# jynik/OOKiedokie

Hardware: NVIDIA B200
Metric: IQ Msamples/s decoded (SC16Q11->OOK msgs) (higher is better)
Workload: dtype f32

## Files before the change

### include/ookd_gpu.h

```cpp
#ifndef OOKD_GPU_H
#define OOKD_GPU_H

#include <stddef.h>
#include <stdint.h>

#ifdef __cplusplus
extern "C" {
#endif

#define OOKD_MAX_STAGES   8
#define OOKD_MAX_TAPS     1024
#define OOKD_MSG_BYTES    32

#define OOKD_OK             0
#define OOKD_ERR_ARG       (-1)
#define OOKD_ERR_CUDA      (-2)
#define OOKD_ERR_NOMEM     (-3)
#define OOKD_ERR_STATE     (-4)
#define OOKD_ERR_OVERFLOW  (-5)

struct ookd_filter_desc {
    uint32_t num_stages;
    uint32_t decimation[OOKD_MAX_STAGES];
    uint32_t num_taps[OOKD_MAX_STAGES];
// ... 38 lines not shown
};

struct ookd_sm_state_k {
    uint32_t first_trigger, num_triggers;
    uint32_t dmin, dmax;
    uint32_t ktimeout;
    uint32_t ksat;
};

struct ookd_sm_compiled {
    uint32_t num_states, num_triggers;
    struct ookd_sm_state_k   *states;
    struct ookd_sm_trigger_k *triggers;
    uint32_t max_bits;
    uint32_t k_sat;
};

int  ookd_sm_compile(const struct ookd_sm_desc *desc, struct ookd_sm_compiled *out);
void ookd_sm_compiled_free(struct ookd_sm_compiled *c);

float ookd_power_threshold(float thr);

extern const int16_t ookd_tune_quarter[257];
int ookd_tune_step(double offset_hz, uint32_t samplerate, uint32_t *step);
int ookd_tune_sc16q11(const int16_t *in, int16_t *out, uint64_t first_sample, uint64_t n_samples, uint32_t step);

struct ookd_msg {
    uint64_t out_sample;
    uint64_t buffer_idx;
    uint32_t num_bits;
    uint32_t reserved;
    uint8_t  data[OOKD_MSG_BYTES];
};

struct ookd_sm_carry {
    uint32_t state;
    uint32_t k;
    uint32_t num_bits;
    uint32_t prev_bit;
    uint8_t  data[OOKD_MSG_BYTES];
};

void ookd_sm_idle_carry(const struct ookd_sm_compiled *c, struct ookd_sm_carry *out);

struct ookd_gpu_config {
    const struct ookd_filter_desc *filter;
    const struct ookd_sm_desc *sm;
    float    threshold;
    uint32_t samples_per_buffer;
    int32_t  device_id;
    uint32_t flags;
    uint32_t sm_chunk_buffers;
    uint32_t sm_warmup;
    uint32_t sm_burst_rounds;
    uint32_t sub_windows;
    uint32_t tune_step;
};

// ... 131 lines not shown
```

### ookiedokie_b200/binding.py

```python
import ctypes as C
import os
import subprocess

import numpy as np

_HERE = os.path.dirname(os.path.abspath(__file__))
LIB_PATH = os.environ.get("OOKD_GPU_LIB") or os.path.join(_HERE, "lib", "libookd_gpu.so")

MAX_STAGES = 8
MSG_BYTES = 32
K_INF = 0xFFFFFFFF

FLAG_FORCE_GENERIC = 1
FLAG_NO_SCREEN = 2
FLAG_NO_TMA = 8
FLAG_SYNC_TAIL = 16
FLAG_SHARE_SMS = 32
FLAG_NO_GRAPH = 64
FLAG_FUSED_SM = 128
FLAG_FMA_SCREEN = 256
FLAG_NO_ADAPTIVE = 512
FLAG_INPUT_CS8 = 1024
FLAG_INPUT_CU8 = 2048

INPUT_FORMATS = {"sc16q11": (0, np.int16), "cs8": (FLAG_INPUT_CS8, np.int8), "cu8": (FLAG_INPUT_CU8, np.uint8)}

EXPORTS = [
    "ookd_sm_compile", "ookd_sm_compiled_free", "ookd_sm_idle_carry", "ookd_power_threshold",
    "ookd_tune_step", "ookd_tune_sc16q11",
    "ookd_gpu_device_count", "ookd_gpu_strerror", "ookd_gpu_last_error",
    "ookd_gpu_create", "ookd_gpu_destroy", "ookd_gpu_decode", "ookd_gpu_decode_shard",
    "ookd_gpu_decode_begin", "ookd_gpu_decode_end", "ookd_gpu_batch_decode",
    "ookd_gpu_resolve", "ookd_gpu_halo", "ookd_gpu_input_bytes", "ookd_gpu_total_decimation", "ookd_gpu_initial_carry",
    "ookd_gpu_edges", "ookd_gpu_bits", "ookd_gpu_filtered", "ookd_gpu_filter_cf", "ookd_gpu_synth", "ookd_gpu_synth_ex",
    "ookd_gpu_host_alloc", "ookd_gpu_host_free", "ookd_gpu_dev_alloc", "ookd_gpu_dev_free",
    "ookd_gpu_memcpy_h2d", "ookd_gpu_memcpy_d2h", "ookd_gpu_filtered_sc16q11",
    "ookd_gpu_multi_create", "ookd_gpu_multi_destroy", "ookd_gpu_multi_halo", "ookd_gpu_multi_n_gpus",
    "ookd_gpu_multi_handle", "ookd_gpu_multi_shards_used", "ookd_gpu_multi_last_error", "ookd_gpu_multi_shard_range",
    "ookd_gpu_multi_decode", "ookd_gpu_multi_edges",
    "ookd_gpu_multi_decode_begin", "ookd_gpu_multi_decode_end", "ookd_gpu_multi_resolve",
]


# ... 25 lines not shown


class SmTriggerK(C.Structure):
    _fields_ = [("cond", C.c_int32), ("action", C.c_int32), ("next_state", C.c_uint32),
                ("kmin", C.c_uint32), ("kmax", C.c_uint32)]


class SmStateK(C.Structure):
    _fields_ = [("first_trigger", C.c_uint32), ("num_triggers", C.c_uint32),
                ("dmin", C.c_uint32), ("dmax", C.c_uint32), ("ktimeout", C.c_uint32), ("ksat", C.c_uint32)]


class SmCompiled(C.Structure):
    _fields_ = [("num_states", C.c_uint32), ("num_triggers", C.c_uint32),
                ("states", C.POINTER(SmStateK)), ("triggers", C.POINTER(SmTriggerK)),
                ("max_bits", C.c_uint32), ("k_sat", C.c_uint32)]


class Msg(C.Structure):
    _fields_ = [("out_sample", C.c_uint64), ("buffer_idx", C.c_uint64), ("num_bits", C.c_uint32),
                ("reserved", C.c_uint32), ("data", C.c_uint8 * MSG_BYTES)]


MSG_DTYPE = np.dtype([("out_sample", "<u8"), ("buffer_idx", "<u8"), ("num_bits", "<u4"), ("reserved", "<u4"),
                      ("data", "u1", (MSG_BYTES,))])
assert MSG_DTYPE.itemsize == C.sizeof(Msg)


def msgs_to_tuples(rec, nbytes):
    return list(zip(rec["out_sample"].tolist(), rec["buffer_idx"].tolist(), rec["num_bits"].tolist(),
                    [bytes(d[:nbytes]) for d in rec["data"]]))
# ... 39 lines not shown


_lib = None


def lib():
    global _lib
    if _lib is None:
        if not os.path.exists(LIB_PATH):
            build_library()
        L = C.CDLL(LIB_PATH)
        L.ookd_sm_compile.restype = C.c_int
        L.ookd_sm_compile.argtypes = [C.POINTER(SmDesc), C.POINTER(SmCompiled)]
        L.ookd_sm_compiled_free.argtypes = [C.POINTER(SmCompiled)]
        L.ookd_sm_idle_carry.argtypes = [C.POINTER(SmCompiled), C.POINTER(SmCarry)]
        L.ookd_power_threshold.restype = C.c_float
        L.ookd_power_threshold.argtypes = [C.c_float]
        L.ookd_tune_step.restype = C.c_int
        L.ookd_tune_step.argtypes = [C.c_double, C.c_uint32, C.POINTER(C.c_uint32)]
        L.ookd_tune_sc16q11.restype = C.c_int
        L.ookd_tune_sc16q11.argtypes = [C.c_void_p, C.c_void_p, C.c_uint64, C.c_uint64, C.c_uint32]
        L.ookd_gpu_device_count.restype = C.c_int
        L.ookd_gpu_strerror.restype = C.c_char_p
        L.ookd_gpu_strerror.argtypes = [C.c_int]
        L.ookd_gpu_last_error.restype = C.c_char_p
        L.ookd_gpu_last_error.argtypes = [C.c_void_p]
        L.ookd_gpu_create.restype = C.c_int
        L.ookd_gpu_create.argtypes = [C.POINTER(C.c_void_p), C.POINTER(GpuConfig)]
        L.ookd_gpu_destroy.argtypes = [C.c_void_p]
        L.ookd_gpu_decode.restype = C.c_int
# ... 130 lines not shown
    return res


def sm_idle_carry(states, num_bits, sample_rate):
    d, keep = make_sm_desc(states, num_bits, sample_rate)
    out = SmCompiled()
    rc = lib().ookd_sm_compile(C.byref(d), C.byref(out))
    if rc != 0:
        raise OokdError(f"ookd_sm_compile: {lib().ookd_gpu_strerror(rc).decode()}")
    c = SmCarry()
    lib().ookd_sm_idle_carry(C.byref(out), C.byref(c))
    lib().ookd_sm_compiled_free(C.byref(out))
    return c.astuple()


def power_threshold(thr):
    return float(lib().ookd_power_threshold(C.c_float(thr)))


def tune_step(offset_hz, samplerate):
    if not 0 <= int(samplerate) < 2**32:
        raise ValueError(f"samplerate {samplerate} is not a uint32")
    step = C.c_uint32()
    if lib().ookd_tune_step(C.c_double(float(offset_hz)), C.c_uint32(int(samplerate)), C.byref(step)) != 0:
        raise ValueError(f"no tune step for an offset of {offset_hz} Hz at {samplerate} samples/s: the offset must be "
                         f"finite and below half the sample rate in magnitude")
    return int(step.value)


def tune_sc16q11(iq, first_sample, step):
# ... 334 lines not shown
```

### ookiedokie_b200/csrc/ookd_gpu.cu

```cuda
#include <cstdarg>
#include <cstdio>
#include <cstdlib>
#include <cmath>
#include <algorithm>
#include <cstring>
#include <mutex>
#include <thread>
#include <type_traits>
#include <vector>

#include "ookd_common.cuh"
#include "fir_kernels.cuh"
#include "screen_tma.cuh"
#include "edge_kernels.cuh"
#include "sm_kernels.cuh"
#include "synth_kernel.cuh"

using namespace ookd;

namespace {

struct DevBuf {
    void  *p = nullptr;
    size_t cap = 0;
// ... 51 lines not shown
    uint32_t tune_step = 0;
    bool screen = false;
    bool screen2 = false;
    bool fma = false;
    bool fma_ok = false;
    bool adaptive = false;
    bool adaptive_ok = false;
    bool fused_sm = true;
    unsigned fused_grid_max = 0;
    unsigned n_sm = 148;

    bool have_sm = false;
    ookd_sm_compiled smc{};
    SmCarry canon{};
    SmTable *d_tab = nullptr;

    DevBuf in, bits, inter[2], block_counts, edges, scalars, chunk_exit[2], chunk_ran, slots, slot_count,
           sm_dbg, slot_off, msgs_dev, dense_list, chunk_e, bound_pos, seed_pos, seed_e, seed_kind, edge_tmp, final_entry, tab_entry, tab_exit, tab_nmsg, tab_cnt[2], tab_link, tab_chosen;
    uint32_t slot_cap = 8;
    bool tables_valid = false;
    int tab_cur = 0;
    bool warmup = false;
    u64 warm_in = 0;
    bool warm = false;
    i64 report_lo = 0;
    SmCarry entry_used{};
    uint32_t first_chunk = 0;
    bool entry_explicit = false;
    void *h_scalars = nullptr;
    SmMsg *h_msgs_pin = nullptr;
// ... 534 lines not shown
        o.buffer_idx = ((m.out_sample + 1) * (u64) h->total_dec - 1) / h->spb;
        o.num_bits = m.num_bits;
        memcpy(o.data, m.data, nbytes);
    }
    if (exit_) carry_from_dev(last, *exit_);
    if (res) {
        res->n_msgs = h->h_msgs.size();
        res->msgs = h->h_msgs.empty() ? nullptr : h->h_msgs.data();
        res->sm_rounds = rounds;
        carry_from_dev(h->entry_used, res->entry_used);
        res->entry_is_provisional = (h->warm && !h->entry_explicit) ? 1u : 0u;
    }
    return OOKD_OK;
}

SmArgs base_sm_args(ookd_gpu *h, const SmCarry &entry0)
{
    SmArgs a{};
    a.tab = h->d_tab;
    a.edges = (const u64 *) h->edges.p;
    a.n_edges = h->n_edges;
    a.base_bit = h->base_bit;
    a.out_lo = h->out_lo; a.out_hi = h->out_hi;
    a.spb = h->spb; a.dec = h->total_dec;
    a.opb = (h->spb % h->total_dec == 0) ? h->spb / h->total_dec : 0;
    a.first_buffer = h->first_buffer;
    a.chunk_buffers = h->chunk_buffers;
    a.n_chunks = h->n_chunks;
    a.entry0 = entry0;
    a.slots = (SmMsg *) h->slots.p;
    a.slot_cap = h->slot_cap;
    a.n_ran = (uint32_t *) ((char *) h->scalars.p + 64);
    a.overflow = (uint32_t *) ((char *) h->scalars.p + 32);
    a.warm = h->warm ? 1u : 0u;
// ... 208 lines not shown
            for (uint32_t r = 0; r < burst; r++) {
                a.round = rounds;
                a.counter_idx = rounds & 31;
                if (rounds == 0) {
                    a.cnt_in = (const uint32_t *) h->tab_cnt[0].p;
                    a.cnt_out = (uint32_t *) h->tab_cnt[0].p;
                } else {
                    CU(h, cudaMemcpyAsync(h->tab_cnt[cur ^ 1].p, h->tab_cnt[cur].p, sizeof(uint32_t) * nc,
                                          cudaMemcpyDeviceToDevice, h->s_compute));
                    a.cnt_in = (const uint32_t *) h->tab_cnt[cur].p;
                    a.cnt_out = (uint32_t *) h->tab_cnt[cur ^ 1].p;
                    cur ^= 1;
                }
                {
                    const u64 warps = (u64) nc * (rounds == 0 ? 1 : TAB_K);
                    sm_table_round_kernel<<<(unsigned) ((warps + SM_ROUND_WARPS - 1) / SM_ROUND_WARPS), 32 * SM_ROUND_WARPS, 0, h->s_compute>>>(a);
                }
                h->launches++;
                CU(h, cudaGetLastError());
                rounds++;
                if (burst == 3 && r <= 1) {
                    a.cnt_in = (const uint32_t *) h->tab_cnt[cur].p;
                    sm_link_kernel<<<(unsigned) (((u64) nc * TAB_K + 127) / 128), 128, 0, h->s_compute>>>(a);
                    sm_walk_kernel<<<1, SM_WALK_NT, 0, h->s_compute>>>(a, nullptr, nullptr, 0, nullptr);
                    h->launches += 2;
                }
            }
            a.cnt_in = (const uint32_t *) h->tab_cnt[cur].p;
            sm_link_kernel<<<(unsigned) (((u64) nc * TAB_K + 127) / 128), 128, 0, h->s_compute>>>(a);
            sm_walk_kernel<<<1, SM_WALK_NT, 0, h->s_compute>>>(a, nullptr, nullptr, 0, nullptr);
            h->launches += 2;
// ... 204 lines not shown
    h->launches++;
    for (uint32_t r = 0; r < h->burst_rounds; r++) {
        a.round = rounds;
        a.counter_idx = rounds & 31;
        if (rounds == 0) {
            a.cnt_in = (const uint32_t *) h->tab_cnt[0].p;
            a.cnt_out = (uint32_t *) h->tab_cnt[0].p;
        } else {
            CU(h, cudaMemcpyAsync(h->tab_cnt[cur ^ 1].p, h->tab_cnt[cur].p, sizeof(uint32_t) * nc, cudaMemcpyDeviceToDevice,
                                  h->s_compute));
            a.cnt_in = (const uint32_t *) h->tab_cnt[cur].p;
            a.cnt_out = (uint32_t *) h->tab_cnt[cur ^ 1].p;
            cur ^= 1;
        }
        const u64 warps = (u64) nc * (rounds == 0 ? 1 : TAB_K);
        sm_table_round_kernel<<<(unsigned) ((warps + SM_ROUND_WARPS - 1) / SM_ROUND_WARPS), 32 * SM_ROUND_WARPS, 0, h->s_compute>>>(a);
        h->launches++;
        CU(h, cudaGetLastError());
        rounds++;
        {
            a.cnt_in = (const uint32_t *) h->tab_cnt[cur].p;
            sm_link_kernel<<<(unsigned) (((u64) nc * TAB_K + 127) / 128), 128, 0, h->s_compute>>>(a);
            sm_walk_kernel<<<1, SM_WALK_NT, 0, h->s_compute>>>(a, (uint32_t *) h->slot_off.p, (SmMsg *) h->msgs_dev.p, msg_cap,
                                                               (u64 *) h->scalars.p + 1);
            h->launches += 2;
        }
    }
    }
    CU(h, cudaGetLastError());
    CU(h, cudaMemcpyAsync(h->h_scalars, h->scalars.p, 352, cudaMemcpyDeviceToHost, h->s_compute));
    if (getenv("OOKD_DEBUG")) {
// ... 136 lines not shown
                us(0), us(1), us(2), us(8), us(9), us(3), us(4), us(5), us(7), rounds, nc);
    }
    if (!h->fused_sm && !h->burst_fixed && overflow == 0 && walk_complete != 1 && h->burst_rounds < 2) {
        h->burst_rounds = 2;
    }
    while (!h->fused_sm && overflow == 0 && walk_complete != 1 && rounds < 16) {
        SmArgs a = fast_sm_args(h, h->pend.e0);
        a.round = rounds;
        a.counter_idx = rounds & 15;
        CU(h, cudaMemcpyAsync(h->tab_cnt[cur ^ 1].p, h->tab_cnt[cur].p, sizeof(uint32_t) * nc, cudaMemcpyDeviceToDevice,
                              h->s_compute));
        a.cnt_in = (const uint32_t *) h->tab_cnt[cur].p;
        a.cnt_out = (uint32_t *) h->tab_cnt[cur ^ 1].p;
        cur ^= 1;
        const u64 warps = (u64) nc * TAB_K;
        sm_table_round_kernel<<<(unsigned) ((warps + SM_ROUND_WARPS - 1) / SM_ROUND_WARPS), 32 * SM_ROUND_WARPS, 0, h->s_compute>>>(a);
        rounds++;
        a.cnt_in = (const uint32_t *) h->tab_cnt[cur].p;
        sm_link_kernel<<<(unsigned) (((u64) nc * TAB_K + 127) / 128), 128, 0, h->s_compute>>>(a);
        sm_walk_kernel<<<1, SM_WALK_NT, 0, h->s_compute>>>(a, nullptr, nullptr, 0, nullptr);
        CU(h, cudaMemcpyAsync(h->slot_off.p, h->slot_count.p, sizeof(uint32_t) * nc, cudaMemcpyDeviceToDevice, h->s_compute));
        scan_u32_kernel<<<1, SCAN_NT, 0, h->s_compute>>>((uint32_t *) h->slot_off.p, nc, (u64 *) h->scalars.p + 1);
        sm_gather_table_kernel<<<(nc + 127) / 128, 128, 0, h->s_compute>>>(a, (const uint32_t *) h->slot_off.p,
                                                                           (SmMsg *) h->msgs_dev.p, msg_cap);
        h->launches += 5;
        CU(h, cudaGetLastError());
        CU(h, cudaMemcpyAsync(h->h_scalars, h->scalars.p, 352, cudaMemcpyDeviceToHost, h->s_compute));
        if (n_copy) {
            CU(h, cudaMemcpyAsync(h->h_msgs_pin, h->msgs_dev.p, sizeof(SmMsg) * n_copy, cudaMemcpyDeviceToHost, h->s_compute));
        }
        if (h->warm) {
// ... 68 lines not shown
    return h ? h->err : "null handle";
}

void ookd_gpu_destroy(ookd_gpu *h)
{
    if (!h) return;
    if (h->sub) ookd_gpu_multi_destroy(h->sub);
    h->sub = nullptr;
    cudaSetDevice(h->device);
    if (h->s_compute) cudaStreamSynchronize(h->s_compute);
    if (h->s_copy) cudaStreamSynchronize(h->s_copy);
    if (h->tail_graph) cudaGraphExecDestroy(h->tail_graph);
    h->tail_graph = nullptr;
    for (auto &st : h->stages) if (st.d_taps) cudaFree(st.d_taps);
    if (h->d_tab) cudaFree(h->d_tab);
    DevBuf *all[] = {&h->in, &h->bits, &h->inter[0], &h->inter[1], &h->block_counts, &h->edges, &h->scalars,
                     &h->chunk_exit[0], &h->chunk_exit[1], &h->chunk_ran, &h->slots, &h->slot_count,
                     &h->sm_dbg, &h->slot_off, &h->msgs_dev, &h->dense_list, &h->chunk_e, &h->bound_pos, &h->seed_pos, &h->seed_e, &h->seed_kind, &h->edge_tmp,
                     &h->final_entry, &h->tab_entry, &h->tab_exit, &h->tab_nmsg, &h->tab_cnt[0],
                     &h->tab_cnt[1], &h->tab_link, &h->tab_chosen};
    for (DevBuf *b : all) release(*b);
    if (h->h_scalars) cudaFreeHost(h->h_scalars);
    if (h->h_msgs_pin) cudaFreeHost(h->h_msgs_pin);
    for (auto e : h->ev_piece) cudaEventDestroy(e);
    if (h->ev_t0) cudaEventDestroy(h->ev_t0);
    if (h->ev_t1) cudaEventDestroy(h->ev_t1);
    if (h->ev_f0) cudaEventDestroy(h->ev_f0);
    if (h->ev_f1) cudaEventDestroy(h->ev_f1);
    if (h->ev_s1) cudaEventDestroy(h->ev_s1);
    if (h->s_compute) cudaStreamDestroy(h->s_compute);
// ... 145 lines not shown
        }
        const int rc = ookd_sm_compile(cfg->sm, &h->smc);
        if (rc != OOKD_OK) CREATE_FAIL(rc);
        SmTable *tab = new SmTable();
        memset(tab, 0, sizeof(*tab));
        tab->num_states = h->smc.num_states;
        tab->num_triggers = h->smc.num_triggers;
        tab->max_bits = h->smc.max_bits;
        tab->k_sat = h->smc.k_sat;
        memcpy(tab->states, h->smc.states, sizeof(ookd_sm_state_k) * h->smc.num_states);
        memcpy(tab->triggers, h->smc.triggers, sizeof(ookd_sm_trigger_k) * h->smc.num_triggers);
        cudaError_t e = cudaMalloc(&h->d_tab, sizeof(SmTable));
        if (e == cudaSuccess) e = cudaMemcpy(h->d_tab, tab, sizeof(SmTable), cudaMemcpyHostToDevice);
        delete tab;
        if (e != cudaSuccess) CREATE_FAIL(OOKD_ERR_CUDA);
        ookd_sm_carry idle;
        ookd_sm_idle_carry(&h->smc, &idle);
        carry_to_dev(idle, h->canon);
        h->have_sm = true;
    }
    if (cfg->sub_windows > 1 && cfg->sm) {
        const uint32_t K = cfg->sub_windows < 16 ? cfg->sub_windows : 16;
        ookd_gpu_config c = *cfg;
        c.sub_windows = 0;
        c.device_id = dev;
        int32_t ids[16];
        for (uint32_t k = 0; k < K; k++) ids[k] = dev;
        const int rc = ookd_gpu_multi_create(&h->sub, &c, ids, K);
        if (rc != OOKD_OK) CREATE_FAIL(rc);
        if (ookd_gpu_multi_halo(h->sub) != h->halo) CREATE_FAIL(OOKD_ERR_STATE);
// ... 606 lines not shown
```

### ookiedokie_b200/csrc/sm_compile.c

```c
#include "ookd_gpu.h"

#include <math.h>
#include <stdlib.h>
#include <string.h>

#define SM_TOLERANCE 0.15
#define K_LIMIT 0x7FFFFFF0u

struct bound {
    double   value;
    int      is_lower;
    uint32_t k;
    int      done;
};

static double win_lo(uint64_t d_us)
{
    const float lo = (float) ((double) d_us - (SM_TOLERANCE * (double) d_us));
    return (double) lo;
}

static double win_hi(uint64_t d_us)
{
    const float hi = (float) ((double) d_us + (SM_TOLERANCE * (double) d_us));
// ... 32 lines not shown
                    b[i].k = k;
                } else {
                    b[i].done = 1;
                    open--;
                }
            }
        }
        if (k >= K_LIMIT) {
            return OOKD_ERR_ARG;
        }
        elapsed += dt;
        k++;
    }
    return OOKD_OK;
}

int ookd_sm_compile(const struct ookd_sm_desc *d, struct ookd_sm_compiled *out)
{
    if (!d || !out || d->num_states == 0 || !d->states || d->max_bits == 0 ||
        d->max_bits > 8 * OOKD_MSG_BYTES || d->sample_rate == 0 ||
        (d->num_triggers != 0 && !d->triggers)) {
        return OOKD_ERR_ARG;
    }
    memset(out, 0, sizeof(*out));

    for (uint32_t s = 0; s < d->num_states; s++) {
        const struct ookd_sm_state_us *st = &d->states[s];
        if ((uint64_t) st->first_trigger + st->num_triggers > d->num_triggers) {
            return OOKD_ERR_ARG;
        }
// ... 86 lines not shown
        struct ookd_sm_state_k *o = &out->states[s];
        for (uint32_t t = 0; t < o->num_triggers; t++) {
            const struct ookd_sm_trigger_k *tk = &out->triggers[o->first_trigger + t];
            if (tk->kmax != OOKD_K_INF) {
                if (tk->kmin + 1 > o->ksat) o->ksat = tk->kmin + 1;
                if (tk->kmax + 1 > o->ksat) o->ksat = tk->kmax + 1;
            }
        }
    }
    free(b);

    out->num_states = d->num_states;
    out->num_triggers = d->num_triggers;
    out->max_bits = d->max_bits;
    out->k_sat = k_max + 1;
    return OOKD_OK;
}

void ookd_sm_compiled_free(struct ookd_sm_compiled *c)
{
    if (c) {
        free(c->states);
        free(c->triggers);
        memset(c, 0, sizeof(*c));
    }
}

float ookd_power_threshold(float thr)
{
    if (isnan(thr)) {
        return thr;
    }
    if (thr <= 0.0f) {
        return 0.0f;
    }
    if (isinf(thr)) {
        return INFINITY;
    }
    float p = thr * thr;
    if (isinf(p)) {
// ... 145 lines not shown
```

### ookiedokie_b200/csrc/sm_kernels.cuh

```cuda
#pragma once

#include "ookd_common.cuh"

namespace ookd {

struct SmDevHdr {
    u64 n_edges;
    uint32_t base_bit, pad;
};

struct SmArgs {
    const SmDevHdr *hdr;
    const SmTable *tab;
    const u64 *edges;
    u64  n_edges;
    uint32_t base_bit;
    i64  out_lo, out_hi;
    u64  spb;
    u64  dec;
    uint32_t opb;
    u64  first_buffer;
    uint32_t chunk_buffers;
    uint32_t n_chunks;
    uint32_t round;
// ... 21 lines not shown
    SmCarry  *final_exit;
    uint32_t *start_slot;
    uint32_t first_chunk;
    uint32_t warm;
    SmCarry  *final_entry;
    i64 report_lo;
    SmCarry  *mid_carry;
    unsigned long long *dbg;
    uint32_t entry_at_report;
    u64 *chunk_e;
    i64 *bound_pos;
    i64 *seed_pos;
    u64 *seed_e;
    uint8_t *seed_kind;
    SmCarry canon;
};

#define OOKD_SEED_TRUE      0
#define OOKD_SEED_CANON     1
#define OOKD_SEED_IDLE      2
#define OOKD_SEED_RESET     3
#define OOKD_SEED_NONE      4

__device__ __forceinline__ i64 first_output_of_buffer(const SmArgs &a, u64 b)
{
    if (a.opb) return (i64) (b * a.opb);
    return (i64) ((b * a.spb) / a.dec);
}

__device__ __forceinline__ u64 buffer_of_output(const SmArgs &a, i64 m)
// ... 300 lines not shown
    if (lane < tab->num_triggers) {
        const ookd_sm_trigger_k t = tab->triggers[lane];
        W.t_cond = (uint32_t) t.cond;
        W.t_pack = (uint32_t) t.action | (t.next_state << 8);
        W.t_kmin = t.kmin; W.t_kmax = t.kmax;
        for (uint32_t st = 0; st < tab->num_states; st++) {
            const ookd_sm_state_k x = tab->states[st];
            if (lane >= x.first_trigger && lane < x.first_trigger + x.num_triggers) {
                W.t_state = st;
                W.s_dmin = x.dmin; W.s_dmax = x.dmax; W.s_ktimeout = x.ktimeout; W.s_ksat = x.ksat;
            }
        }
    }
}

__device__ __forceinline__ int warp_sm_apply(const WarpSm &W, SmCarry &s, uint32_t pack)
{
    const uint32_t action = pack & 0xFFu;
    int result = 0;
    if (action == OOKD_ACT_APPEND_0 || action == OOKD_ACT_APPEND_1) {
        if (s.num_bits <= W.max_bits && s.num_bits < 256) {
            const u64 m = 1ull << (s.num_bits & 63);
            const u64 set = (action == OOKD_ACT_APPEND_1) ? m : 0ull;
            if (s.num_bits < 64) {
                s.data[0] = (s.data[0] & ~m) | set;
            } else {
                const uint32_t w = s.num_bits >> 6;
#pragma unroll
                for (uint32_t i = 1; i < 4; i++) {
                    if (i == w) s.data[i] = (s.data[i] & ~m) | set;
                }
            }
        }
        s.num_bits++;
    } else if (action == OOKD_ACT_OUTPUT_DATA) {
        result = 1;
    }
    s.state = pack >> 8;
    return result;
}

__device__ __forceinline__ int warp_sm_eval(const WarpSm &W, SmCarry &s, uint32_t b)
{
    const uint32_t k = s.k;
    const bool rise = !s.prev && b, fall = s.prev && !b;
    const bool cond_ok = (W.t_cond == OOKD_COND_ALWAYS) || (W.t_cond == OOKD_COND_PULSE_START && rise) ||
                         (W.t_cond == OOKD_COND_PULSE_END && fall) ||
                         (W.t_cond == OOKD_COND_TIMEOUT && W.s_ktimeout != OOKD_K_INF && k >= W.s_ktimeout) ||
                         (W.t_cond == OOKD_COND_MSG_COMPLETE && s.num_bits >= W.max_bits);
    const bool elig = (W.t_state == s.state) && k >= W.t_kmin && k <= W.t_kmax && cond_ok;
    const uint32_t mask = __ballot_sync(0xFFFFFFFFu, elig);
    if (mask == 0) {
        const uint32_t ksat = __shfl_sync(0xFFFFFFFFu, W.ksat_by_state, (int) s.state);
        s.k = (k + 1 < ksat) ? k + 1 : ksat;
// ... 550 lines not shown
    bool live = c < a.n_chunks;
    if (live && a.round != 0) live = (c != 0) && j < a.cnt_in[c - 1];
    if (threadIdx.x == 0) s_any = 0;
    __syncthreads();
    if (live && lane == 0) s_any = 1;
    __syncthreads();
    if (!s_any) return;
    load_table(T, a.tab);
    if (!live) return;
    const bool capable = warp_sm_supported(a.tab);
    WarpSm W;
    if (capable) warp_sm_load(W, &T, lane);
    sm_round_pair(a, T, W, capable, c, j, lane, n_edges, base_bit);
}

__global__ void __launch_bounds__(32) sm_table_add_entry_kernel(const SmArgs a)
{
    __shared__ SmTable T;
    load_table(T, a.tab);
    const uint32_t lane = threadIdx.x & 31;
    const uint32_t K = a.tab_k;
    const uint32_t c = a.first_chunk;
    const uint32_t n_here = a.cnt_out[c];
    SmCarry s = a.entry0;
    if (!a.entry_at_report) {
        for (uint32_t i = 0; i < n_here; i++) {
            if (carry_equal(s, a.tab_entry[(u64) c * K + i])) { if (lane == 0) *a.start_slot = i; return; }
        }
    } else {
        for (uint32_t i = 0; i < n_here; i++) {
// ... 417 lines not shown
```

Baseline: 1.001 million.

## Add precompiled breakpoint table and per-thread state machine evaluation

Compiles the OOK state machine into a per-state breakpoint table that gives, for each k interval, the quiet-fire time and the rising/falling edge outcomes. A new kernel runs one chunk/entry pair per thread, with the table copied into shared memory, instead of one warp per pair using ballot-based trigger evaluation. Long runs with no edge are skipped in a single step by jumping straight to the next fire time. This cuts per-sample and per-warp cost in the sequential state-machine rounds. In exchange, only one pair is packed per thread, which can cause divergence, and lookups add shared-memory traffic; machines with too many states or breakpoints fall back to the old warp path.

```diff
diff --git a/include/ookd_gpu.h b/include/ookd_gpu.h
--- a/include/ookd_gpu.h
+++ b/include/ookd_gpu.h
@@ -76,7 +76,15 @@
     struct ookd_sm_trigger_k *triggers;
     uint32_t max_bits;
     uint32_t k_sat;
-};
+    uint32_t *table;
+    uint32_t table_words;
+};
+
+#define OOKD_SMT_MAX_STATES 32
+#define OOKD_SMT_BP         16
+#define OOKD_SMT_ROW        (OOKD_SMT_BP * 9)
+#define OOKD_SMT_ERROR      0xFFFFFFFFu
+#define OOKD_SMT_MAX_WORDS  (OOKD_SMT_MAX_STATES * OOKD_SMT_ROW)
 
 int  ookd_sm_compile(const struct ookd_sm_desc *desc, struct ookd_sm_compiled *out);
 void ookd_sm_compiled_free(struct ookd_sm_compiled *c);
@@ -104,6 +112,9 @@
 };
 
 void ookd_sm_idle_carry(const struct ookd_sm_compiled *c, struct ookd_sm_carry *out);
+
+int ookd_sm_table_step(const struct ookd_sm_compiled *c, struct ookd_sm_carry *s, uint32_t b);
+uint32_t ookd_sm_table_quiet(const struct ookd_sm_compiled *c, const struct ookd_sm_carry *s, uint32_t *k_fire);
 
 struct ookd_gpu_config {
     const struct ookd_filter_desc *filter;
diff --git a/ookiedokie_b200/binding.py b/ookiedokie_b200/binding.py
--- a/ookiedokie_b200/binding.py
+++ b/ookiedokie_b200/binding.py
@@ -8,6 +8,9 @@
 LIB_PATH = os.environ.get("OOKD_GPU_LIB") or os.path.join(_HERE, "lib", "libookd_gpu.so")
 
 MAX_STAGES = 8
+SMT_BP = 16
+SMT_ROW = SMT_BP * 9
+SMT_ERROR = 0xFFFFFFFF
 MSG_BYTES = 32
 K_INF = 0xFFFFFFFF
 
@@ -26,7 +29,8 @@
 INPUT_FORMATS = {"sc16q11": (0, np.int16), "cs8": (FLAG_INPUT_CS8, np.int8), "cu8": (FLAG_INPUT_CU8, np.uint8)}
 
 EXPORTS = [
-    "ookd_sm_compile", "ookd_sm_compiled_free", "ookd_sm_idle_carry", "ookd_power_threshold",
+    "ookd_sm_compile", "ookd_sm_compiled_free", "ookd_sm_idle_carry", "ookd_sm_table_step", "ookd_sm_table_quiet",
+    "ookd_power_threshold",
     "ookd_tune_step", "ookd_tune_sc16q11",
     "ookd_gpu_device_count", "ookd_gpu_strerror", "ookd_gpu_last_error",
     "ookd_gpu_create", "ookd_gpu_destroy", "ookd_gpu_decode", "ookd_gpu_decode_shard",
@@ -82,7 +86,8 @@
 class SmCompiled(C.Structure):
     _fields_ = [("num_states", C.c_uint32), ("num_triggers", C.c_uint32),
                 ("states", C.POINTER(SmStateK)), ("triggers", C.POINTER(SmTriggerK)),
-                ("max_bits", C.c_uint32), ("k_sat", C.c_uint32)]
+                ("max_bits", C.c_uint32), ("k_sat", C.c_uint32),
+                ("table", C.POINTER(C.c_uint32)), ("table_words", C.c_uint32)]
 
 
 class Msg(C.Structure):
@@ -152,6 +157,10 @@
         L.ookd_sm_compile.argtypes = [C.POINTER(SmDesc), C.POINTER(SmCompiled)]
         L.ookd_sm_compiled_free.argtypes = [C.POINTER(SmCompiled)]
         L.ookd_sm_idle_carry.argtypes = [C.POINTER(SmCompiled), C.POINTER(SmCarry)]
+        L.ookd_sm_table_step.restype = C.c_int
+        L.ookd_sm_table_step.argtypes = [C.POINTER(SmCompiled), C.POINTER(SmCarry), C.c_uint32]
+        L.ookd_sm_table_quiet.restype = C.c_uint32
+        L.ookd_sm_table_quiet.argtypes = [C.POINTER(SmCompiled), C.POINTER(SmCarry), C.POINTER(C.c_uint32)]
         L.ookd_power_threshold.restype = C.c_float
         L.ookd_power_threshold.argtypes = [C.c_float]
         L.ookd_tune_step.restype = C.c_int
@@ -312,6 +321,41 @@
     return c.astuple()
 
 
+class CompiledSm:
+
+    def __init__(self, states, num_bits, sample_rate):
+        d, keep = make_sm_desc(states, num_bits, sample_rate)
+        self.c = SmCompiled()
+        rc = lib().ookd_sm_compile(C.byref(d), C.byref(self.c))
+        if rc != 0:
+            self.c = None
+            raise OokdError(f"ookd_sm_compile: {lib().ookd_gpu_strerror(rc).decode()}")
+
+    def table(self):
+        if not self.c.table:
+            return None
+        return np.ctypeslib.as_array(self.c.table, shape=(self.c.table_words,)).copy().reshape(self.c.num_states, -1)
+
+    def ksat(self, s):
+        return self.c.states[s].ksat
+
+    def step(self, carry, b):
+        x = SmCarry.fromtuple(carry)
+        r = lib().ookd_sm_table_step(C.byref(self.c), C.byref(x), int(b))
+        return r, x.astuple()
+
+    def quiet(self, carry):
+        x = SmCarry.fromtuple(carry)
+        k = C.c_uint32(0)
+        pack = lib().ookd_sm_table_quiet(C.byref(self.c), C.byref(x), C.byref(k))
+        return pack, k.value
+
+    def __del__(self):
+        if getattr(self, "c", None) is not None and lib is not None:
+            lib().ookd_sm_compiled_free(C.byref(self.c))
+            self.c = None
+
+
 def power_threshold(thr):
     return float(lib().ookd_power_threshold(C.c_float(thr)))
 
diff --git a/ookiedokie_b200/csrc/ookd_gpu.cu b/ookiedokie_b200/csrc/ookd_gpu.cu
--- a/ookiedokie_b200/csrc/ookd_gpu.cu
+++ b/ookiedokie_b200/csrc/ookd_gpu.cu
@@ -89,6 +89,9 @@
     ookd_sm_compiled smc{};
     SmCarry canon{};
     SmTable *d_tab = nullptr;
+    uint32_t *d_smt = nullptr;
+    uint32_t smt_words = 0;
+    uint32_t smt_ppw = 32;
 
     DevBuf in, bits, inter[2], block_counts, edges, scalars, chunk_exit[2], chunk_ran, slots, slot_count,
            sm_dbg, slot_off, msgs_dev, dense_list, chunk_e, bound_pos, seed_pos, seed_e, seed_kind, edge_tmp, final_entry, tab_entry, tab_exit, tab_nmsg, tab_cnt[2], tab_link, tab_chosen;
@@ -653,10 +656,23 @@
     return OOKD_OK;
 }
 
+void launch_round(ookd_gpu *h, const SmArgs &a, u64 pairs)
+{
+    if (h->d_smt) {
+        sm_thread_round_kernel<<<(unsigned) ((pairs + a.smt_ppw - 1) / a.smt_ppw), SM_THREAD_NT,
+                                 sizeof(uint32_t) * h->smt_words, h->s_compute>>>(a);
+    } else {
+        sm_table_round_kernel<<<(unsigned) ((pairs + SM_ROUND_WARPS - 1) / SM_ROUND_WARPS), 32 * SM_ROUND_WARPS, 0, h->s_compute>>>(a);
+    }
+}
+
 SmArgs base_sm_args(ookd_gpu *h, const SmCarry &entry0)
 {
     SmArgs a{};
     a.tab = h->d_tab;
+    a.smt = h->d_smt;
+    a.smt_words = h->smt_words;
+    a.smt_ppw = h->smt_ppw;
     a.edges = (const u64 *) h->edges.p;
     a.n_edges = h->n_edges;
     a.base_bit = h->base_bit;
@@ -895,7 +911,7 @@
                 }
                 {
                     const u64 warps = (u64) nc * (rounds == 0 ? 1 : TAB_K);
-                    sm_table_round_kernel<<<(unsigned) ((warps + SM_ROUND_WARPS - 1) / SM_ROUND_WARPS), 32 * SM_ROUND_WARPS, 0, h->s_compute>>>(a);
+                    launch_round(h, a, warps);
                 }
                 h->launches++;
                 CU(h, cudaGetLastError());
@@ -1130,7 +1146,7 @@
             cur ^= 1;
         }
         const u64 warps = (u64) nc * (rounds == 0 ? 1 : TAB_K);
-        sm_table_round_kernel<<<(unsigned) ((warps + SM_ROUND_WARPS - 1) / SM_ROUND_WARPS), 32 * SM_ROUND_WARPS, 0, h->s_compute>>>(a);
+        launch_round(h, a, warps);
         h->launches++;
         CU(h, cudaGetLastError());
         rounds++;
@@ -1297,7 +1313,7 @@
         a.cnt_out = (uint32_t *) h->tab_cnt[cur ^ 1].p;
         cur ^= 1;
         const u64 warps = (u64) nc * TAB_K;
-        sm_table_round_kernel<<<(unsigned) ((warps + SM_ROUND_WARPS - 1) / SM_ROUND_WARPS), 32 * SM_ROUND_WARPS, 0, h->s_compute>>>(a);
+        launch_round(h, a, warps);
         rounds++;
         a.cnt_in = (const uint32_t *) h->tab_cnt[cur].p;
         sm_link_kernel<<<(unsigned) (((u64) nc * TAB_K + 127) / 128), 128, 0, h->s_compute>>>(a);
@@ -1396,6 +1412,7 @@
     h->tail_graph = nullptr;
     for (auto &st : h->stages) if (st.d_taps) cudaFree(st.d_taps);
     if (h->d_tab) cudaFree(h->d_tab);
+    if (h->d_smt) cudaFree(h->d_smt);
     DevBuf *all[] = {&h->in, &h->bits, &h->inter[0], &h->inter[1], &h->block_counts, &h->edges, &h->scalars,
                      &h->chunk_exit[0], &h->chunk_exit[1], &h->chunk_ran, &h->slots, &h->slot_count,
                      &h->sm_dbg, &h->slot_off, &h->msgs_dev, &h->dense_list, &h->chunk_e, &h->bound_pos, &h->seed_pos, &h->seed_e, &h->seed_kind, &h->edge_tmp,
@@ -1571,6 +1588,17 @@
         if (e == cudaSuccess) e = cudaMemcpy(h->d_tab, tab, sizeof(SmTable), cudaMemcpyHostToDevice);
         delete tab;
         if (e != cudaSuccess) CREATE_FAIL(OOKD_ERR_CUDA);
+        const char *ev = getenv("OOKD_SM_EVAL");
+        if (h->smc.table && !(ev && strcmp(ev, "warp") == 0)) {
+            e = cudaMalloc(&h->d_smt, sizeof(uint32_t) * h->smc.table_words);
+            if (e == cudaSuccess) {
+                e = cudaMemcpy(h->d_smt, h->smc.table, sizeof(uint32_t) * h->smc.table_words, cudaMemcpyHostToDevice);
+            }
+            if (e != cudaSuccess) CREATE_FAIL(OOKD_ERR_CUDA);
+            h->smt_words = h->smc.table_words;
+            const char *ppw = getenv("OOKD_SM_PPW");
+            if (ppw && atoi(ppw) >= 1 && atoi(ppw) <= 32) h->smt_ppw = (uint32_t) atoi(ppw);
+        }
         ookd_sm_carry idle;
         ookd_sm_idle_carry(&h->smc, &idle);
         carry_to_dev(idle, h->canon);
diff --git a/ookiedokie_b200/csrc/sm_compile.c b/ookiedokie_b200/csrc/sm_compile.c
--- a/ookiedokie_b200/csrc/sm_compile.c
+++ b/ookiedokie_b200/csrc/sm_compile.c
@@ -70,6 +70,8 @@
     }
     return OOKD_OK;
 }
+
+static int build_table(struct ookd_sm_compiled *c);
 
 int ookd_sm_compile(const struct ookd_sm_desc *d, struct ookd_sm_compiled *out)
 {
@@ -186,6 +188,10 @@
     out->num_triggers = d->num_triggers;
     out->max_bits = d->max_bits;
     out->k_sat = k_max + 1;
+    if (build_table(out) != OOKD_OK) {
+        ookd_sm_compiled_free(out);
+        return OOKD_ERR_NOMEM;
+    }
     return OOKD_OK;
 }
 
@@ -194,8 +200,209 @@
     if (c) {
         free(c->states);
         free(c->triggers);
+        free(c->table);
         memset(c, 0, sizeof(*c));
     }
+}
+
+
+static uint32_t tab_outcome(const struct ookd_sm_compiled *c, uint32_t s, uint32_t k, uint32_t prev, uint32_t b, int mc)
+{
+    const struct ookd_sm_state_k *st = &c->states[s];
+    for (uint32_t i = 0; i < st->num_triggers; i++) {
+        const struct ookd_sm_trigger_k *t = &c->triggers[st->first_trigger + i];
+        if (k < t->kmin || k > t->kmax) {
+            continue;
+        }
+        int fire = 0, check = 0;
+        switch (t->cond) {
+            case OOKD_COND_ALWAYS:       fire = 1; break;
+            case OOKD_COND_PULSE_START:  fire = check = (!prev && b); break;
+            case OOKD_COND_PULSE_END:    fire = check = (prev && !b); break;
+            case OOKD_COND_TIMEOUT:      fire = (st->ktimeout != OOKD_K_INF && k >= st->ktimeout); break;
+            case OOKD_COND_MSG_COMPLETE: fire = mc; break;
+            default: break;
+        }
+        if (fire) {
+            if (check && !(k >= st->dmin && k <= st->dmax)) {
+                return OOKD_SMT_ERROR;
+            }
+            return (uint32_t) t->action | (t->next_state << 8);
+        }
+    }
+    return 0;
+}
+
+static uint32_t tab_quiet(const struct ookd_sm_compiled *c, uint32_t s, uint32_t k, int mc, uint32_t *L)
+{
+    const struct ookd_sm_state_k *st = &c->states[s];
+    uint32_t best_k = OOKD_K_INF, pack = 0;
+    for (uint32_t i = 0; i < st->num_triggers; i++) {
+        const struct ookd_sm_trigger_k *t = &c->triggers[st->first_trigger + i];
+        uint32_t lo = t->kmin;
+        if (t->cond == OOKD_COND_TIMEOUT) {
+            if (st->ktimeout == OOKD_K_INF) continue;
+            if (st->ktimeout > lo) lo = st->ktimeout;
+        } else if (t->cond == OOKD_COND_MSG_COMPLETE) {
+            if (!mc) continue;
+        } else if (t->cond != OOKD_COND_ALWAYS) {
+            continue;
+        }
+        const uint32_t kk = lo > k ? lo : k;
+        if (kk > t->kmax) continue;
+        if (kk < best_k) {
+            best_k = kk;
+            pack = (uint32_t) t->action | (t->next_state << 8);
+        }
+    }
+    *L = best_k;
+    return pack;
+}
+
+static void bp_add(uint32_t *bp, uint32_t *n, uint32_t v, uint32_t ksat)
+{
+    if (v == 0 || v > ksat || v == OOKD_K_INF) {
+        return;
+    }
+    for (uint32_t i = 0; i < *n; i++) {
+        if (bp[i] == v) return;
+    }
+    if (*n < 2 * 32 + 4) {
+        bp[(*n)++] = v;
+    }
+}
+
+static int cmp_u32(const void *x, const void *y)
+{
+    const uint32_t a = *(const uint32_t *) x, b = *(const uint32_t *) y;
+    return (a > b) - (a < b);
+}
+
+static int build_table(struct ookd_sm_compiled *c)
+{
+    c->table = NULL;
+    c->table_words = 0;
+    if (c->num_states > OOKD_SMT_MAX_STATES || c->num_triggers > 32) {
+        return OOKD_OK;
+    }
+    uint32_t *tab = malloc(sizeof(uint32_t) * OOKD_SMT_ROW * c->num_states);
+    if (!tab) {
+        return OOKD_ERR_NOMEM;
+    }
+    for (uint32_t s = 0; s < c->num_states; s++) {
+        const struct ookd_sm_state_k *st = &c->states[s];
+        uint32_t bp[2 * 32 + 4], n = 0;
+        const uint32_t ksat = st->ksat;
+        bp_add(bp, &n, st->ktimeout, ksat);
+        bp_add(bp, &n, st->dmin, ksat);
+        if (st->dmax != OOKD_K_INF) bp_add(bp, &n, st->dmax + 1, ksat);
+        for (uint32_t i = 0; i < st->num_triggers; i++) {
+            const struct ookd_sm_trigger_k *t = &c->triggers[st->first_trigger + i];
+            bp_add(bp, &n, t->kmin, ksat);
+            if (t->kmax != OOKD_K_INF) bp_add(bp, &n, t->kmax + 1, ksat);
+        }
+        if (n > OOKD_SMT_BP - 1) {
+            free(tab);
+            return OOKD_OK;
+        }
+        qsort(bp, n, sizeof(bp[0]), cmp_u32);
+        uint32_t *row = tab + (size_t) s * OOKD_SMT_ROW;
+        row[0] = ksat;
+        for (uint32_t j = 1; j < OOKD_SMT_BP; j++) {
+            row[j] = (j - 1 < n) ? bp[j - 1] : OOKD_K_INF;
+        }
+        for (uint32_t i = 0; i < OOKD_SMT_BP; i++) {
+            uint32_t *o = row + OOKD_SMT_BP + 8 * i;
+            if (i > n) {
+                memset(o, 0, 8 * sizeof(uint32_t));
+                continue;
+            }
+            const uint32_t k = (i == 0) ? 0 : bp[i - 1];
+            for (int mc = 0; mc < 2; mc++) {
+                uint32_t L;
+                const uint32_t pack = tab_quiet(c, s, k, mc, &L);
+                o[2 * mc] = pack ? L : OOKD_K_INF;
+                o[2 * mc + 1] = pack;
+                o[4 + mc] = tab_outcome(c, s, k, 0, 1, mc);
+                o[6 + mc] = tab_outcome(c, s, k, 1, 0, mc);
+            }
+        }
+    }
+    c->table = tab;
+    c->table_words = OOKD_SMT_ROW * c->num_states;
+    return OOKD_OK;
+}
+
+static const uint32_t *tab_interval(const struct ookd_sm_compiled *c, uint32_t s, uint32_t k)
+{
+    const uint32_t *row = c->table + (size_t) s * OOKD_SMT_ROW;
+    uint32_t i = 0;
+    for (uint32_t j = 1; j < OOKD_SMT_BP; j++) {
+        i += (row[j] <= k);
+    }
+    return row + OOKD_SMT_BP + 8 * i;
+}
+
+static int tab_eval(const struct ookd_sm_compiled *c, struct ookd_sm_carry *s, uint32_t b)
+{
+    const uint32_t *o = tab_interval(c, s->state, s->k);
+    const int mc = s->num_bits >= c->max_bits;
+    uint32_t pack;
+    if ((s->prev_bit & 1u) == b) {
+        pack = (o[2 * mc] <= s->k) ? o[2 * mc + 1] : 0;
+    } else {
+        pack = o[(b ? 4 : 6) + mc];
+    }
+    if (pack == 0) {
+        const uint32_t ksat = c->table[(size_t) s->state * OOKD_SMT_ROW];
+        s->k = (s->k + 1 < ksat) ? s->k + 1 : ksat;
+        return 0;
+    }
+    s->k = 0;
+    if (pack == OOKD_SMT_ERROR) {
+        s->state = 0;
+        return -1;
+    }
+    const uint32_t action = pack & 0xFFu;
+    int result = 0;
+    if (action == OOKD_ACT_APPEND_0 || action == OOKD_ACT_APPEND_1) {
+        if (s->num_bits <= c->max_bits && s->num_bits < 8 * OOKD_MSG_BYTES) {
+            const uint32_t byte = s->num_bits >> 3, bit = s->num_bits & 7;
+            if (action == OOKD_ACT_APPEND_1) s->data[byte] |= (uint8_t) (1u << bit);
+            else s->data[byte] &= (uint8_t) ~(1u << bit);
+        }
+        s->num_bits++;
+    } else if (action == OOKD_ACT_OUTPUT_DATA) {
+        result = 1;
+    }
+    s->state = pack >> 8;
+    return result;
+}
+
+int ookd_sm_table_step(const struct ookd_sm_compiled *c, struct ookd_sm_carry *s, uint32_t b)
+{
+    int r = 0;
+    b &= 1u;
+    if (s->state == 0) {
+        const uint32_t nbytes = (c->max_bits + 7) / 8;
+        s->num_bits = 0;
+        memset(s->data, 0, nbytes < OOKD_MSG_BYTES ? nbytes : OOKD_MSG_BYTES);
+        r = tab_eval(c, s, b);
+    }
+    if (r == 0) {
+        r = tab_eval(c, s, b);
+    }
+    s->prev_bit = b;
+    return r;
+}
+
+uint32_t ookd_sm_table_quiet(const struct ookd_sm_compiled *c, const struct ookd_sm_carry *s, uint32_t *k_fire)
+{
+    const uint32_t *o = tab_interval(c, s->state, s->k);
+    const int mc = s->num_bits >= c->max_bits;
+    const uint32_t L = o[2 * mc], pack = o[2 * mc + 1];
+    *k_fire = pack ? (L > s->k ? L : s->k) : OOKD_K_INF;
+    return pack;
 }
 
 float ookd_power_threshold(float thr)
diff --git a/ookiedokie_b200/csrc/sm_kernels.cuh b/ookiedokie_b200/csrc/sm_kernels.cuh
--- a/ookiedokie_b200/csrc/sm_kernels.cuh
+++ b/ookiedokie_b200/csrc/sm_kernels.cuh
@@ -59,6 +59,9 @@
     u64 *seed_e;
     uint8_t *seed_kind;
     SmCarry canon;
+    const uint32_t *smt;
+    uint32_t smt_words;
+    uint32_t smt_ppw;
 };
 
 #define OOKD_SEED_TRUE      0
@@ -389,12 +392,12 @@
     }
 }
 
-__device__ __forceinline__ int warp_sm_apply(const WarpSm &W, SmCarry &s, uint32_t pack)
+__device__ __forceinline__ int sm_apply_pack(const uint32_t max_bits, SmCarry &s, uint32_t pack)
 {
     const uint32_t action = pack & 0xFFu;
     int result = 0;
     if (action == OOKD_ACT_APPEND_0 || action == OOKD_ACT_APPEND_1) {
-        if (s.num_bits <= W.max_bits && s.num_bits < 256) {
+        if (s.num_bits <= max_bits && s.num_bits < 256) {
             const u64 m = 1ull << (s.num_bits & 63);
             const u64 set = (action == OOKD_ACT_APPEND_1) ? m : 0ull;
             if (s.num_bits < 64) {
@@ -413,6 +416,11 @@
     }
     s.state = pack >> 8;
     return result;
+}
+
+__device__ __forceinline__ int warp_sm_apply(const WarpSm &W, SmCarry &s, uint32_t pack)
+{
+    return sm_apply_pack(W.max_bits, s, pack);
 }
 
 __device__ __forceinline__ int warp_sm_eval(const WarpSm &W, SmCarry &s, uint32_t b)
@@ -993,6 +1001,402 @@
     sm_round_pair(a, T, W, capable, c, j, lane, n_edges, base_bit);
 }
 
+struct SmtRow {
+    uint32_t w[OOKD_SMT_BP];
+};
+
+__device__ __forceinline__ void smt_row(const uint32_t *smt, uint32_t state, SmtRow &r)
+{
+    const uint4 *p = (const uint4 *) (smt + state * OOKD_SMT_ROW);
+#pragma unroll
+    for (int i = 0; i < OOKD_SMT_BP / 4; i++) {
+        const uint4 v = p[i];
+        r.w[4 * i] = v.x; r.w[4 * i + 1] = v.y; r.w[4 * i + 2] = v.z; r.w[4 * i + 3] = v.w;
+    }
+}
+
+__device__ __forceinline__ uint32_t smt_interval(const SmtRow &r, uint32_t k)
+{
+    uint32_t i = 0;
+#pragma unroll
+    for (int j = 1; j < OOKD_SMT_BP; j++) i += (r.w[j] <= k) ? 1u : 0u;
+    return i;
+}
+
+__device__ __forceinline__ int thr_sm_eval(const uint32_t *smt, uint32_t max_bits, SmCarry &s, uint32_t b)
+{
+    SmtRow r;
+    smt_row(smt, s.state, r);
+    const uint32_t k = s.k;
+    const uint32_t mc = (s.num_bits >= max_bits) ? 1u : 0u;
+    const uint32_t *o = smt + s.state * OOKD_SMT_ROW + OOKD_SMT_BP + 8 * smt_interval(r, k);
+    uint32_t pack;
+    if (s.prev == b) {
+        const uint2 q = *(const uint2 *) (o + 2 * mc);
+        pack = (q.x <= k) ? q.y : 0u;
+    } else {
+        pack = o[(b ? 4 : 6) + mc];
+    }
+    if (pack == 0) {
+        s.k = (k + 1 < r.w[0]) ? k + 1 : r.w[0];
+        return 0;
+    }
+    s.k = 0;
+    if (pack == OOKD_SMT_ERROR) {
+        s.state = 0;
+        return -1;
+    }
+    return sm_apply_pack(max_bits, s, pack);
+}
+
+__device__ __forceinline__ int thr_sm_step(const uint32_t *smt, uint32_t max_bits, SmCarry &s, uint32_t b)
+{
+    int r = 0;
+    if (s.state == 0) {
+        s.num_bits = 0;
+        const uint32_t nbytes = (max_bits + 7) >> 3;
+#pragma unroll
+        for (int w = 0; w < 4; w++) {
+            const uint32_t lo = 8u * w;
+            if (nbytes >= lo + 8) {
+                s.data[w] = 0;
+            } else if (nbytes > lo) {
+                s.data[w] &= ~((1ull << (8 * (nbytes - lo))) - 1);
+            }
+        }
+        r = thr_sm_eval(smt, max_bits, s, b);
+    }
+    if (r == 0) {
+        r = thr_sm_eval(smt, max_bits, s, b);
+    }
+    s.prev = b;
+    return r;
+}
+
+struct ThrEdges {
+    const u64 *edges;
+    u64 n_edges, ebase, org;
+    uint32_t A[8];
+    u64 R[8];
+
+    __device__ __forceinline__ uint32_t off(u64 v) const
+    {
+        const u64 d = v - org;
+        return d < 0xFFFFFFFFull ? (uint32_t) d : 0xFFFFFFFFu;
+    }
+    __device__ __forceinline__ void fetch8(u64 idx, u64 (&r)[8]) const
+    {
+        if (idx + 8 <= n_edges) {
+            const ulonglong2 *p = (const ulonglong2 *) (edges + idx);
+#pragma unroll
+            for (int i = 0; i < 4; i++) {
+                const ulonglong2 v = p[i];
+                r[2 * i] = v.x;
+                r[2 * i + 1] = v.y;
+            }
+        } else {
+#pragma unroll
+            for (int i = 0; i < 8; i++) r[i] = (idx + i < n_edges) ? edges[idx + i] : org + 0xFFFFFFFFull;
+        }
+    }
+    __device__ __forceinline__ void reset(u64 e)
+    {
+        ebase = e & ~1ull;
+        fetch8(ebase, R);
+#pragma unroll
+        for (int i = 0; i < 8; i++) A[i] = off(R[i]);
+        fetch8(ebase + 8, R);
+    }
+    __device__ __forceinline__ uint32_t at(u64 e)
+    {
+        if (e - ebase >= 8) {
+            if (e - ebase >= 16) {
+                reset(e);
+            } else {
+#pragma unroll
+                for (int i = 0; i < 8; i++) A[i] = off(R[i]);
+                ebase += 8;
+                fetch8(ebase + 8, R);
+            }
+        }
+        const uint32_t d = (uint32_t) (e - ebase);
+        uint32_t v = A[0];
+#pragma unroll
+        for (int i = 1; i < 8; i++) v = (d == (uint32_t) i) ? A[i] : v;
+        return v;
+    }
+    __device__ __forceinline__ u64 first_at_or_after(u64 e, uint32_t nb, u64 nb64)
+    {
+        if (e - ebase < 16) {
+            const uint32_t d = (uint32_t) (e - ebase);
+            uint32_t n = 0;
+#pragma unroll
+            for (int i = 0; i < 8; i++) {
+                n += ((uint32_t) i >= d && A[i] < nb ? 1u : 0u) + ((uint32_t) i + 8 >= d && off(R[i]) < nb ? 1u : 0u);
+            }
+            if (off(R[7]) >= nb) return e + n;
+            const u64 from = ebase + 16;
+            return from + edge_lower_bound_near(edges + from, n_edges - from, nb64);
+        }
+        return e + edge_lower_bound_near(edges + e, n_edges - e, nb64);
+    }
+};
+
+__device__ __forceinline__ void thr_sm_run_span(const SmArgs &a, const u64 n_edges, const uint32_t *smt, const uint32_t max_bits,
+                                                SmCarry &s, i64 pos64, i64 end64, u64 e, uint32_t tb, SpanOut &o, i64 chunk_lo)
+{
+    uint32_t pos = (uint32_t) (pos64 - chunk_lo);
+    const uint32_t end = (uint32_t) (end64 - chunk_lo);
+    ThrEdges E;
+    E.edges = a.edges; E.n_edges = n_edges; E.org = (u64) chunk_lo;
+    E.reset(e);
+    uint32_t next_edge = E.at(e);
+
+    if (s.prev & OOKD_CARRY_DROPPING) {
+        s.prev &= 1u;
+        i64 nb64 = next_buffer_start(a, pos64, chunk_lo);
+        const bool more = nb64 > end64;
+        if (more) nb64 = end64;
+        const uint32_t nb = (uint32_t) (nb64 - chunk_lo);
+        if (next_edge < nb) {
+            const u64 e2 = E.first_at_or_after(e, nb, (u64) nb64);
+            tb ^= (uint32_t) ((e2 - e) & 1);
+            e = e2;
+            next_edge = E.at(e);
+        }
+        pos = nb;
+        if (more) s.prev |= OOKD_CARRY_DROPPING;
+    }
+
+    while (pos < end) {
+        o.steps++;
+        int r;
+        if (s.state == 0 || s.prev != tb) {
+            const bool at_edge = (next_edge == pos);
+            const uint32_t b = at_edge ? (tb ^ 1u) : tb;
+            o.singles++;
+            r = thr_sm_step(smt, max_bits, s, b);
+            if (at_edge) {
+                tb ^= 1u;
+                e++;
+                next_edge = E.at(e);
+            }
+            pos++;
+        } else {
+            const bool have_edge = next_edge < end;
+            const uint32_t limit = have_edge ? next_edge : end;
+            const uint32_t g = limit - pos;
+            const uint32_t k = s.k;
+            const uint32_t b = tb ^ 1u;
+            SmtRow row;
+            smt_row(smt, s.state, row);
+            const uint32_t ksat = row.w[0];
+            const uint32_t k_e = min(k + g, ksat);
+            const uint32_t mc = (s.num_bits >= max_bits) ? 1u : 0u;
+            const uint32_t *o8 = smt + s.state * OOKD_SMT_ROW + OOKD_SMT_BP;
+            const uint2 q = *(const uint2 *) (o8 + 8 * smt_interval(row, k) + 2 * mc);
+            const uint32_t ew = o8[8 * smt_interval(row, k_e) + (b ? 4 : 6) + mc];
+            const uint32_t tau = max(q.x, k) - k;
+            if (q.y != 0 && tau < g) {
+                pos += tau + 1;
+                s.k = 0;
+                r = sm_apply_pack(max_bits, s, q.y);
+            } else if (!have_edge || ew == 0) {
+                const u64 kn = (u64) k + g + (have_edge ? 1u : 0u);
+                s.k = (kn < (u64) ksat) ? (uint32_t) kn : ksat;
+                pos = limit;
+                if (have_edge) {
+                    s.prev = b;
+                    tb ^= 1u;
+                    e++;
+                    next_edge = E.at(e);
+                    pos++;
+                }
+                continue;
+            } else {
+                s.k = 0;
+                if (ew == OOKD_SMT_ERROR) {
+                    s.state = 0;
+                    r = -1;
+                } else {
+                    r = sm_apply_pack(max_bits, s, ew);
+                }
+                s.prev = b;
+                tb ^= 1u;
+                e++;
+                next_edge = E.at(e);
+                pos = limit + 1;
+            }
+        }
+        if (r > 0) {
+            sm_emit(o, s, chunk_lo + (i64) pos - 1);
+        } else if (r < 0) {
+            o.errs++;
+            i64 nb64 = next_buffer_start(a, chunk_lo + (i64) pos - 1, chunk_lo);
+            if (nb64 > end64) {
+                nb64 = end64;
+                s.prev |= OOKD_CARRY_DROPPING;
+            }
+            const uint32_t nb = (uint32_t) (nb64 - chunk_lo);
+            if (nb > pos) {
+                if (next_edge < nb) {
+                    const u64 e2 = E.first_at_or_after(e, nb, (u64) nb64);
+                    tb ^= (uint32_t) ((e2 - e) & 1);
+                    e = e2;
+                    next_edge = E.at(e);
+                }
+                pos = nb;
+            }
+        }
+    }
+}
+
+__device__ __forceinline__ void sm_round_pair_thread(const SmArgs &a, const SmTable &T, const uint32_t *smt, uint32_t c, uint32_t j,
+                                                     const u64 n_edges, const uint32_t base_bit)
+{
+    const uint32_t K = a.tab_k;
+    const uint32_t max_bits = T.max_bits;
+    i64 start, end, lo;
+    chunk_bounds(a, c, start, end, lo);
+    const bool fits = (end - lo) < (1ll << 31);
+
+    u64 e = a.chunk_e[c];
+    uint32_t tb = base_bit ^ (uint32_t) (e & 1);
+
+    SmCarry s, entry;
+    i64 pos = start;
+    uint32_t slot;
+    if (a.round == 0) {
+        const uint32_t kind = a.seed_kind[c];
+        if (kind == OOKD_SEED_NONE) return;
+        pos = a.seed_pos[c];
+        e = a.seed_e[c];
+        tb = base_bit ^ (uint32_t) (e & 1);
+        if (kind == OOKD_SEED_TRUE) {
+            s = a.entry_ptr ? *a.entry_ptr : a.entry0;
+            if (s.state < T.num_states && s.k > T.states[s.state].ksat) s.k = T.states[s.state].ksat;
+        } else if (kind == OOKD_SEED_CANON || kind == OOKD_SEED_IDLE) {
+            s = a.canon;
+        } else {
+            carry_reset(s, tb);
+        }
+        entry = s;
+        slot = 0;
+    } else {
+        if (c == 0) return;
+        const uint32_t n_prev = a.cnt_in[c - 1];
+        if (j >= n_prev) return;
+        s = a.tab_exit[(u64) (c - 1) * K + j];
+        for (uint32_t i = 0; i < j; i++) {
+            if (carry_equal(s, a.tab_exit[(u64) (c - 1) * K + i])) return;
+        }
+        const uint32_t n_here = a.cnt_in[c];
+        for (uint32_t i = 0; i < n_here; i++) {
+            if (carry_equal(s, a.tab_entry[(u64) c * K + i])) return;
+        }
+        slot = atomicAdd(&a.cnt_out[c], 1u);
+        if (slot >= K) {
+            atomicExch(a.overflow, 2u);
+            return;
+        }
+        entry = s;
+    }
+    atomicAdd(&a.n_ran[a.counter_idx], 1u);
+
+    uint32_t cc = c;
+    const long long t_dbg = a.dbg ? clock64() : 0;
+    for (int hop = 0;; hop++) {
+        SpanOut o;
+        o.slots = a.slots + ((u64) cc * K + slot) * a.slot_cap;
+        o.cap = a.slot_cap;
+        o.n_msgs = 0;
+        o.overflow = a.overflow;
+        i64 upto = end;
+        const bool through_report = a.warm && cc == 0 && pos < a.report_lo && a.report_lo <= end;
+        if (through_report) upto = a.report_lo;
+        if (fits) {
+            thr_sm_run_span(a, n_edges, smt, max_bits, s, pos, upto, e, tb, o, lo);
+        } else {
+            sm_run_span<false>(a, n_edges, T, s, pos, upto, e, tb, o, lo);
+        }
+        if (through_report) {
+            a.mid_carry[slot] = s;
+            if (upto < end) {
+                e = edge_lower_bound(a.edges, n_edges, (u64) upto);
+                tb = base_bit ^ (uint32_t) (e & 1);
+                if (fits) {
+                    thr_sm_run_span(a, n_edges, smt, max_bits, s, upto, end, e, tb, o, lo);
+                } else {
+                    sm_run_span<false>(a, n_edges, T, s, upto, end, e, tb, o, lo);
+                }
+            }
+        }
+        a.tab_entry[(u64) cc * K + slot] = entry;
+        a.tab_exit[(u64) cc * K + slot] = s;
+        a.tab_nmsg[(u64) cc * K + slot] = (o.n_msgs < o.cap) ? o.n_msgs : o.cap;
+        if (a.dbg && a.round == 0) {
+            a.dbg[(u64) c * 4 + 0] = (unsigned long long) (clock64() - t_dbg);
+            a.dbg[(u64) c * 4 + 1] += o.steps;
+            a.dbg[(u64) c * 4 + 2] += ((unsigned long long) o.errs << 32) | o.singles;
+            a.dbg[(u64) c * 4 + 3] = (unsigned long long) hop + 1;
+        }
+        if (!fits || hop >= 16 || cc + 1 >= a.n_chunks) return;
+        const uint32_t nn = cc + 1;
+        bool known = false;
+        if (a.round == 0) {
+            const uint32_t kind = a.seed_kind[nn];
+            if (kind == OOKD_SEED_CANON || kind == OOKD_SEED_IDLE) {
+                known = carry_equal(s, a.canon);
+            } else if (kind == OOKD_SEED_RESET) {
+                SmCarry r;
+                carry_reset(r, base_bit ^ (uint32_t) (a.seed_e[nn] & 1));
+                known = carry_equal(s, r);
+            }
+        } else {
+            const uint32_t n_next = a.cnt_in[nn];
+            for (uint32_t i = 0; i < n_next; i++) {
+                if (carry_equal(s, a.tab_entry[(u64) nn * K + i])) { known = true; break; }
+            }
+        }
+        if (known) return;
+        const uint32_t nslot = atomicAdd(&a.cnt_out[nn], 1u);
+        if (nslot >= K) {
+            atomicExch(a.overflow, 2u);
+            return;
+        }
+        atomicAdd(&a.n_ran[a.counter_idx], 1u);
+        cc = nn;
+        slot = nslot;
+        entry = s;
+        chunk_bounds(a, cc, start, end, lo);
+        if ((end - lo) >= (1ll << 31)) return;
+        pos = start;
+        e = a.chunk_e[cc];
+        tb = base_bit ^ (uint32_t) (e & 1);
+    }
+}
+
+constexpr int SM_THREAD_NT = 32;
+
+__global__ void __launch_bounds__(SM_THREAD_NT) sm_thread_round_kernel(const SmArgs a)
+{
+    OOKD_SM_EDGE_HDR(a)
+    __shared__ SmTable T;
+    extern __shared__ __align__(16) uint32_t s_smt[];
+    const uint32_t K = a.tab_k;
+    const uint32_t KR = (a.round == 0) ? 1u : K;
+    const uint32_t gid = blockIdx.x * a.smt_ppw + threadIdx.x;
+    const uint32_t c = gid / KR, j = gid % KR;
+    if (a.round >= 1 && a.walk_status[1]) return;
+    bool live = threadIdx.x < a.smt_ppw && c < a.n_chunks;
+    if (live && a.round != 0) live = (c != 0) && j < a.cnt_in[c - 1];
+    if (!__syncthreads_or(live)) return;
+    for (uint32_t i = threadIdx.x; i < a.smt_words; i += SM_THREAD_NT) s_smt[i] = a.smt[i];
+    load_table(T, a.tab);
+    if (!live) return;
+    sm_round_pair_thread(a, T, s_smt, c, j, n_edges, base_bit);
+}
+
 __global__ void __launch_bounds__(32) sm_table_add_entry_kernel(const SmArgs a)
 {
     __shared__ SmTable T;
```

Result: slower. 975,400 (median of 6 runs) (-2.6%).
